# meyerls/PEGASUS

Hardware: AMD Instinct MI355X
Metric: rendered views/sec (RGB+depth+mask) on 2M-Gaussian scene @800x800 (higher is better)
Workload: dtype f32

## Files before the change

### pegasus_amd/csrc/preprocess.hip.h

```cpp
#pragma once
#include "blockcull.hip.h"
#include "pgr_common.h"

namespace pgr {

__device__ __forceinline__ float dot3_chain(float a0, float b0, float a1, float b1, float a2, float b2) {
    return fmaf(a2, b2, fmaf(a1, b1, a0 * b0));
}

__device__ __forceinline__ int clamp_trunc(float f, int hi) {
    if (!(f > 0.0f)) return 0;
    if (f >= (float)hi) return hi;
    return (int)f;
}

struct TileRect { int minx, miny, maxx, maxy; };

__device__ __forceinline__ TileRect tile_rect(float px, float py, int radius, int grid_x, int grid_y) {
    const float rf = (float)radius;
    TileRect r;
    r.minx = clamp_trunc((px - rf) / (float)TILE, grid_x);
    r.miny = clamp_trunc((py - rf) / (float)TILE, grid_y);
    r.maxx = clamp_trunc((px + rf + (float)(TILE - 1)) / (float)TILE, grid_x);
    r.maxy = clamp_trunc((py + rf + (float)(TILE - 1)) / (float)TILE, grid_y);
    return r;
}

__device__ __forceinline__ void cov3d_from_scale_rot(float s0, float s1, float s2, float mod, float4 q, float cov[6]) {
    const float r = q.x, x = q.y, y = q.z, z = q.w;
    float R[3][3];
    R[0][0] = 1.0f - 2.0f * (y * y + z * z);
    R[0][1] = 2.0f * (x * y - r * z);
    R[0][2] = 2.0f * (x * z + r * y);
    R[1][0] = 2.0f * (x * y + r * z);
    R[1][1] = 1.0f - 2.0f * (x * x + z * z);
    R[1][2] = 2.0f * (y * z - r * x);
    R[2][0] = 2.0f * (x * z - r * y);
    R[2][1] = 2.0f * (y * z + r * x);
    R[2][2] = 1.0f - 2.0f * (x * x + y * y);
    const float sx = mod * s0, sy = mod * s1, sz = mod * s2;
    float M[3][3];
#pragma unroll
    for (int i = 0; i < 3; ++i) {
        M[i][0] = R[i][0] * sx;
        M[i][1] = R[i][1] * sy;
        M[i][2] = R[i][2] * sz;
    }
    cov[0] = dot3_chain(M[0][0], M[0][0], M[0][1], M[0][1], M[0][2], M[0][2]);
    cov[1] = dot3_chain(M[0][0], M[1][0], M[0][1], M[1][1], M[0][2], M[1][2]);
    cov[2] = dot3_chain(M[0][0], M[2][0], M[0][1], M[2][1], M[0][2], M[2][2]);
    cov[3] = dot3_chain(M[1][0], M[1][0], M[1][1], M[1][1], M[1][2], M[1][2]);
    cov[4] = dot3_chain(M[1][0], M[2][0], M[1][1], M[2][1], M[1][2], M[2][2]);
    cov[5] = dot3_chain(M[2][0], M[2][0], M[2][1], M[2][1], M[2][2], M[2][2]);
}

template <int DEG>
__device__ __forceinline__ void sh_basis(float x, float y, float z, float b[16]) {
    constexpr float C0 = 0.28209479177387814f;
    constexpr float C1 = 0.4886025119029199f;
    constexpr float C2_0 = 1.0925484305920792f, C2_1 = -1.0925484305920792f, C2_2 = 0.31539156525252005f,
                    C2_3 = -1.0925484305920792f, C2_4 = 0.5462742152960396f;
    constexpr float C3_0 = -0.5900435899266435f, C3_1 = 2.890611442640554f, C3_2 = -0.4570457994644658f,
                    C3_3 = 0.3731763325901154f, C3_4 = -0.4570457994644658f, C3_5 = 1.445305721320277f,
                    C3_6 = -0.5900435899266435f;
    b[0] = C0;
    if constexpr (DEG > 0) {
        b[1] = -(C1 * y);
        b[2] = C1 * z;
        b[3] = -(C1 * x);
    }
    if constexpr (DEG > 1) {
        const float xx = x * x, yy = y * y, zz = z * z;
        const float xy = x * y, yz = y * z, xz = x * z;
        b[4] = C2_0 * xy;
        b[5] = C2_1 * yz;
        b[6] = C2_2 * (2.0f * zz - xx - yy);
        b[7] = C2_3 * xz;
        b[8] = C2_4 * (xx - yy);
        if constexpr (DEG > 2) {
            b[9] = C3_0 * y * (3.0f * xx - yy);
            b[10] = C3_1 * xy * z;
            b[11] = C3_2 * y * (4.0f * zz - xx - yy);
            b[12] = C3_3 * z * (2.0f * zz - 3.0f * xx - 3.0f * yy);
            b[13] = C3_4 * x * (4.0f * zz - xx - yy);
            b[14] = C3_5 * z * (xx - yy);
            b[15] = C3_6 * x * (xx - 3.0f * yy);
        }
    }
}

template <int DEG>
__device__ __forceinline__ float3 sh_to_rgb(const float* __restrict__ sh, float dx, float dy, float dz) {
    float b[16];
    sh_basis<DEG>(dx, dy, dz, b);
    constexpr int NC = (DEG + 1) * (DEG + 1);
    float acc[3];
    acc[0] = b[0] * sh[0];
    acc[1] = b[0] * sh[1];
    acc[2] = b[0] * sh[2];
#pragma unroll
    for (int k = 1; k < NC; ++k) {
        acc[0] = fmaf(b[k], sh[3 * k + 0], acc[0]);
        acc[1] = fmaf(b[k], sh[3 * k + 1], acc[1]);
        acc[2] = fmaf(b[k], sh[3 * k + 2], acc[2]);
    }
    return make_float3(fmaxf(acc[0] + 0.5f, 0.0f), fmaxf(acc[1] + 0.5f, 0.0f), fmaxf(acc[2] + 0.5f, 0.0f));
}

__device__ __forceinline__ uint2 candidate_rect(const TileRect& r, float mx, float my, float c_xx, float c_yy,
                                                float con_x, float con_y, float con_z, float opacity, int radius) {
    if (opacity < ALPHA_MIN) return make_uint2(0u, 0u);
    const uint2 full = make_uint2((uint32_t)r.minx | ((uint32_t)r.miny << 16), (uint32_t)r.maxx | ((uint32_t)r.maxy << 16));
    if (!(con_x > 0.0f) || !(con_z > 0.0f)) return full;
    const float t = 255.0f * opacity;
    const uint32_t bits = __float_as_uint(t);
    const float e = (float)((int)((bits >> 23) & 0xffu) - 127);
    const float m = __uint_as_float((bits & 0x007fffffu) | 0x3f800000u);
    const float tau = 1.3862944f * (e + (m - 1.0f) + 0.0861f);
    const float D = (float)radius + 2.0f * (float)TILE;
    const float M = (con_x + 2.0f * fabsf(con_y) + con_z) * D * D;
    const float tau2 = 1.001f * (tau + 0.00001f * M + 0.01f) + 0.001f;
    const float ex = sqrtf(tau2 * c_xx) * 1.001f + 1.0f, ey = sqrtf(tau2 * c_yy) * 1.001f + 1.0f;
    if (!(ex < 1.0e9f) || !(ey < 1.0e9f)) return full;
    const int minx = max(r.minx, (int)floorf((mx - ex - (float)(TILE - 1)) / (float)TILE) + 0);
    const int miny = max(r.miny, (int)floorf((my - ey - (float)(TILE - 1)) / (float)TILE) + 0);
    const int maxx = min(r.maxx, (int)floorf((mx + ex) / (float)TILE) + 1);
    const int maxy = min(r.maxy, (int)floorf((my + ey) / (float)TILE) + 1);
    if (maxx <= minx || maxy <= miny) return make_uint2(0u, 0u);
    return make_uint2((uint32_t)minx | ((uint32_t)miny << 16), (uint32_t)maxx | ((uint32_t)maxy << 16));
}

constexpr int SPLAT_F4 = 3;

struct PreOut {
    float4* splats;
    uint2* rects;
    uint2* crects;
    int32_t* radii;
};

struct ShRegs { float v[48]; };

template <int DEG>
__device__ __forceinline__ float3 sh_regs_to_rgb(const ShRegs& sh, float dx, float dy, float dz) {
    float b[16];
    sh_basis<DEG>(dx, dy, dz, b);
    constexpr int NC = (DEG + 1) * (DEG + 1);
    float acc[3];
    acc[0] = b[0] * sh.v[0];
    acc[1] = b[0] * sh.v[1];
    acc[2] = b[0] * sh.v[2];
#pragma unroll
    for (int k = 1; k < NC; ++k) {
        acc[0] = fmaf(b[k], sh.v[3 * k + 0], acc[0]);
        acc[1] = fmaf(b[k], sh.v[3 * k + 1], acc[1]);
        acc[2] = fmaf(b[k], sh.v[3 * k + 2], acc[2]);
    }
    return make_float3(fmaxf(acc[0] + 0.5f, 0.0f), fmaxf(acc[1] + 0.5f, 0.0f), fmaxf(acc[2] + 0.5f, 0.0f));
}

template <int DEG>
__device__ __forceinline__ void load_sh(ShRegs& sh, const float* __restrict__ p, bool vec4) {
    constexpr int NF = 3 * (DEG + 1) * (DEG + 1);
    if (vec4 && NF % 4 == 0) {
#pragma unroll
        for (int k = 0; k < NF / 4; ++k) {
            const float4 q = reinterpret_cast<const float4*>(p)[k];
            sh.v[4 * k + 0] = q.x; sh.v[4 * k + 1] = q.y; sh.v[4 * k + 2] = q.z; sh.v[4 * k + 3] = q.w;
        }
    } else {
#pragma unroll
        for (int k = 0; k < NF; ++k) sh.v[k] = p[k];
    }
}

typedef float f32x3_a4 __attribute__((ext_vector_type(3), aligned(4)));
typedef float f32x4_a4 __attribute__((ext_vector_type(4), aligned(4)));
template <int DEG>
__device__ __forceinline__ void load_sh_split(ShRegs& sh, const float* __restrict__ dc, const float* __restrict__ rest) {
    constexpr int NR = 3 * ((DEG + 1) * (DEG + 1) - 1);
    const f32x3_a4 c0 = *reinterpret_cast<const f32x3_a4*>(dc);
    sh.v[0] = c0.x; sh.v[1] = c0.y; sh.v[2] = c0.z;
#pragma unroll
    for (int k = 0; k < NR / 4; ++k) {
        const f32x4_a4 q = *reinterpret_cast<const f32x4_a4*>(rest + 4 * k);
        sh.v[3 + 4 * k + 0] = q.x; sh.v[3 + 4 * k + 1] = q.y; sh.v[3 + 4 * k + 2] = q.z; sh.v[3 + 4 * k + 3] = q.w;
    }
#pragma unroll
    for (int k = NR / 4 * 4; k < NR; ++k) sh.v[3 + k] = rest[k];
}

constexpr int POSE_STRIDE = 20;
struct PosedDev {
    const int32_t* object_id;
    const float* poses;
    int32_t k;
};

struct LayerDev {
    const int32_t* layer_id;
    int32_t n_layers;
};

template <int DEG, bool POSED, bool LAYERED = false, bool SPLIT_SH = false>
__global__ __launch_bounds__(PRE_BLOCK) __attribute__((amdgpu_waves_per_eu(4, 4))) void preprocess_batch_kernel(PgrScene sc, const CameraDev* __restrict__ cams,
                                                                     const PreOut* __restrict__ outs, int n_views,
                                                                     PosedDev posed, uint32_t* __restrict__ vis_out,
                                                                     int vis_words, LayerDev layers = LayerDev{nullptr, 0},
                                                                     int views_per_block = 0x7fffffff) {
    const int i = blockIdx.x * PRE_BLOCK + threadIdx.x;
    const int lane = threadIdx.x & (WAVE - 1);
    if (i - lane >= sc.n) return;
    const bool real = i < sc.n;
    const int group = __builtin_amdgcn_readfirstlane(i / WAVE);
    BlockBounds bounds;
    if (vis_out) bounds = wave_block_bounds(sc, i, real, POSED ? posed.object_id : nullptr);
    unsigned long long vis_mask = ~0ull;
    const float bx = real ? sc.means3d[3 * i + 0] : 0.f, by = real ? sc.means3d[3 * i + 1] : 0.f,
                bz = real ? sc.means3d[3 * i + 2] : 0.f;
    const int oid = POSED && real ? posed.object_id[i] : 0;
    int layer = 0;
    if (LAYERED && real) {
        layer = layers.layer_id[i];
        if (layer < 0 || layer > layers.n_layers) layer = 0;
    }
    float cov[6];
    bool have_cov = false, have_sh = false;
    ShRegs sh;
    const bool vec4 = (sc.sh_stride * 3) % 4 == 0 && (reinterpret_cast<uintptr_t>(sc.shs) & 15u) == 0;

    const int v_begin = (int)blockIdx.y * views_per_block;
    const int v_end = (int)min((long long)n_views, (long long)v_begin + views_per_block);
    for (int v = v_begin; v < v_end; ++v) {
        const CameraDev& cam = cams[v];
        const PreOut& o = outs[v];
        if (vis_out) {
            if ((v & (WAVE - 1)) == 0) {
                const int view = v + lane;
                vis_mask = __ballot(view < n_views && !block_is_culled(bounds, cams[view]));
                if (lane == 0) {
                    vis_out[(size_t)group * vis_words + (v >> 5)] = (uint32_t)vis_mask;
                    if ((v >> 5) + 1 < vis_words) vis_out[(size_t)group * vis_words + (v >> 5) + 1] = (uint32_t)(vis_mask >> 32);
                }
            }
            if (!((vis_mask >> (v & (WAVE - 1))) & 1ull)) {
                if (real && o.radii) o.radii[i] = 0;
                if (real && o.rects) o.rects[i] = make_uint2(0u, 0u);
                continue;
            }
        }
        if (!real) continue;
        if (LAYERED && layer == 0) {
            if (o.radii) o.radii[i] = 0;
            if (o.rects) o.rects[i] = make_uint2(0u, 0u);
            o.crects[i] = make_uint2(0u, 0u);
            continue;
        }
        int radius = 0;
        uint2 rect = make_uint2(0u, 0u), crect = make_uint2(0u, 0u);
        float vm[16];
#pragma unroll
        for (int k = 0; k < 16; ++k) vm[k] = cam.view[k];
        const float* pm = cam.proj;
        float cam_cx = cam.campos[0], cam_cy = cam.campos[1], cam_cz = cam.campos[2];
        float cam_tanx = cam.tanfovx, cam_tany = cam.tanfovy, cam_fx = cam.focal_x, cam_fy = cam.focal_y;
        int cam_w = cam.width, cam_h = cam.height, cam_gx = cam.grid_x, cam_gy = cam.grid_y;
        float4* out_splats = o.splats;
        uint2* out_crects = o.crects;
        asm volatile("" : "+s"(out_splats), "+s"(out_crects));
#pragma unroll
        for (int k = 0; k < 15; ++k)
            if ((k & 3) != 3) asm volatile("" : "+s"(vm[k]));
        asm volatile("" : "+s"(cam_cx), "+s"(cam_cy), "+s"(cam_cz), "+s"(cam_tanx), "+s"(cam_tany), "+s"(cam_fx), "+s"(cam_fy));
        asm volatile("" : "+s"(cam_w), "+s"(cam_h), "+s"(cam_gx), "+s"(cam_gy));
        float px = bx, py = by, pz = bz;
        const float* P = nullptr;
        if (POSED && oid > 0) {
            P = posed.poses + ((size_t)v * posed.k + (size_t)(oid - 1)) * POSE_STRIDE;
            const float dx = bx - P[12], dy = by - P[13], dz = bz - P[14];
            px = fmaf(P[2], dz, fmaf(P[1], dy, P[0] * dx)) + P[12] + P[9];
            py = fmaf(P[5], dz, fmaf(P[4], dy, P[3] * dx)) + P[13] + P[10];
            pz = fmaf(P[8], dz, fmaf(P[7], dy, P[6] * dx)) + P[14] + P[11];
        }
        float tx = vm[0] * px + vm[4] * py + vm[8] * pz + vm[12];
        float ty = vm[1] * px + vm[5] * py + vm[9] * pz + vm[13];
        const float tz = vm[2] * px + vm[6] * py + vm[10] * pz + vm[14];
        if (tz > NEAR_Z) {
            const float hx = pm[0] * px + pm[4] * py + pm[8] * pz + pm[12];
            const float hy = pm[1] * px + pm[5] * py + pm[9] * pz + pm[13];
            const float hw = pm[3] * px + pm[7] * py + pm[11] * pz + pm[15];
            const float p_w = 1.0f / (hw + 0.0000001f);
            const float ndc_x = hx * p_w, ndc_y = hy * p_w;
            if (POSED && P) {
                const float4 q = reinterpret_cast<const float4*>(sc.rotations)[i];
                const float inv = 1.0f / fmaxf(sqrtf(q.x * q.x + q.y * q.y + q.z * q.z + q.w * q.w), 1e-12f);
                const float w = q.x * inv, x = q.y * inv, y = q.z * inv, z = q.w * inv;
                const float a = P[15], b = P[16], c = P[17], d = P[18];
                const float4 qp = make_float4(a * w - b * x - c * y - d * z, a * x + b * w + c * z - d * y,
                                              a * y - b * z + c * w + d * x, a * z + b * y - c * x + d * w);
                cov3d_from_scale_rot(sc.scales[3 * i + 0], sc.scales[3 * i + 1], sc.scales[3 * i + 2],
                                     sc.scale_modifier, qp, cov);
            } else if (!have_cov) {
                if (sc.cov3d_precomp) {
#pragma unroll
                    for (int k = 0; k < 6; ++k) cov[k] = sc.cov3d_precomp[6 * (size_t)i + k];
                } else {
                    const float4 q = reinterpret_cast<const float4*>(sc.rotations)[i];
                    cov3d_from_scale_rot(sc.scales[3 * i + 0], sc.scales[3 * i + 1], sc.scales[3 * i + 2],
                                         sc.scale_modifier, q, cov);
                }
                have_cov = true;
            }
            const float limx = 1.3f * cam_tanx, limy = 1.3f * cam_tany;
            const float txtz = tx / tz, tytz = ty / tz;
            tx = fminf(limx, fmaxf(-limx, txtz)) * tz;
            ty = fminf(limy, fmaxf(-limy, tytz)) * tz;
            const float j00 = cam_fx / tz;
            const float j02 = -(cam_fx * tx) / (tz * tz);
            const float j11 = cam_fy / tz;
            const float j12 = -(cam_fy * ty) / (tz * tz);
            float T0[3], T1[3];
#pragma unroll
            for (int c = 0; c < 3; ++c) {
                T0[c] = fmaf(j02, vm[4 * c + 2], j00 * vm[4 * c + 0]);
                T1[c] = fmaf(j12, vm[4 * c + 2], j11 * vm[4 * c + 1]);
            }
            const float S[3][3] = {{cov[0], cov[1], cov[2]}, {cov[1], cov[3], cov[4]}, {cov[2], cov[4], cov[5]}};
            float U0[3], U1[3];
#pragma unroll
            for (int c = 0; c < 3; ++c) {
                U0[c] = dot3_chain(T0[0], S[0][c], T0[1], S[1][c], T0[2], S[2][c]);
                U1[c] = dot3_chain(T1[0], S[0][c], T1[1], S[1][c], T1[2], S[2][c]);
            }
            const float c_xx = dot3_chain(U0[0], T0[0], U0[1], T0[1], U0[2], T0[2]) + LOWPASS;
            const float c_xy = dot3_chain(U0[0], T1[0], U0[1], T1[1], U0[2], T1[2]);
            const float c_yy = dot3_chain(U1[0], T1[0], U1[1], T1[1], U1[2], T1[2]) + LOWPASS;
            const float det = c_xx * c_yy - c_xy * c_xy;
            if (det != 0.0f) {
                const float det_inv = 1.0f / det;
                const float con_x = c_yy * det_inv, con_y = -c_xy * det_inv, con_z = c_xx * det_inv;
                const float mid = 0.5f * (c_xx + c_yy);
                const float disc = sqrtf(fmaxf(0.1f, mid * mid - det));
                const float lambda1 = mid + disc, lambda2 = mid - disc;
                const float rad_f = ceilf(3.0f * sqrtf(fmaxf(lambda1, lambda2)));
                const int rad = rad_f >= 2147483520.0f ? 2147483520 : (int)rad_f;
                const float pix_x = ((ndc_x + 1.0f) * (float)cam_w - 1.0f) * 0.5f;
                const float pix_y = ((ndc_y + 1.0f) * (float)cam_h - 1.0f) * 0.5f;
                const TileRect r = tile_rect(pix_x, pix_y, rad, cam_gx, cam_gy);
                const int w = r.maxx - r.minx, h = r.maxy - r.miny;
                if (w > 0 && h > 0) {
                    float3 rgb;
                    if (sc.colors_precomp) {
                        rgb = make_float3(sc.colors_precomp[3 * (size_t)i], sc.colors_precomp[3 * (size_t)i + 1],
                                          sc.colors_precomp[3 * (size_t)i + 2]);
                    } else {
                        if (!have_sh) {
                            if constexpr (SPLIT_SH)
                                load_sh_split<DEG>(sh, sc.shs + (size_t)i * 3, sc.shs_rest + (size_t)i * (sc.sh_stride - 1) * 3);
                            else
                                load_sh<DEG>(sh, sc.shs + (size_t)i * sc.sh_stride * 3, vec4);
                            have_sh = true;
                        }
                        float dx = px - cam_cx, dy = py - cam_cy, dz = pz - cam_cz;
                        const float len = sqrtf(dx * dx + dy * dy + dz * dz);
                        dx = dx / len; dy = dy / len; dz = dz / len;
                        if (POSED && P) {
                            const float ox = fmaf(P[6], dz, fmaf(P[3], dy, P[0] * dx));
                            const float oy = fmaf(P[7], dz, fmaf(P[4], dy, P[1] * dx));
                            const float oz = fmaf(P[8], dz, fmaf(P[5], dy, P[2] * dx));
                            dx = ox; dy = oy; dz = oz;
                        }
                        rgb = sh_regs_to_rgb<DEG>(sh, dx, dy, dz);
                    }
                    radius = rad;
                    rect = make_uint2((uint32_t)r.minx | ((uint32_t)r.miny << 16),
                                      (uint32_t)r.maxx | ((uint32_t)r.maxy << 16));
                    const float op = sc.opacities[i];
                    crect = candidate_rect(r, pix_x, pix_y, c_xx, c_yy, con_x, con_y, con_z, op, rad);
                    if (LAYERED) {
                        const uint32_t off = (uint32_t)((layer - 1) * cam_gy) << 16;
                        rect.x += off; rect.y += off;
                        if (crect.x | crect.y) { crect.x += off; crect.y += off; }
                    }
                    float4* rec = out_splats + (size_t)i * SPLAT_F4;
                    rec[0] = make_float4(pix_x, pix_y, con_x, con_y);
                    rec[1] = make_float4(con_z, op, con_y / con_z, con_y / con_x);
                    rec[2] = make_float4(rgb.x, rgb.y, rgb.z, tz);
                }
            }
        }
        if (o.radii) o.radii[i] = radius;
        if (o.rects) o.rects[i] = rect;
        out_crects[i] = crect;
    }
}

constexpr int CAM_PACK_MAX = 32;
struct CamPack {
    const float* view[CAM_PACK_MAX];
    const float* proj[CAM_PACK_MAX];
    const float* campos[CAM_PACK_MAX];
    const float* bg[CAM_PACK_MAX];
    float tanfovx[CAM_PACK_MAX], tanfovy[CAM_PACK_MAX];
    int32_t depth_mode[CAM_PACK_MAX];
};

__device__ __forceinline__ void pack_camera(const CamPack& p, int v, int t, int width, int height, CameraDev* __restrict__ out) {
    if (t < 16) {
        out->view[t] = p.view[v][t];
        out->proj[t] = p.proj[v][t];
    }
    if (t < 3) {
        out->campos[t] = p.campos[v][t];
        out->bg[t] = p.bg[v][t];
    }
    if (t == 0) {
        const float tanfovx = p.tanfovx[v], tanfovy = p.tanfovy[v];
        out->tanfovx = tanfovx;
        out->tanfovy = tanfovy;
        out->focal_x = (float)width / (2.0f * tanfovx);
        out->focal_y = (float)height / (2.0f * tanfovy);
        out->width = width;
        out->height = height;
        out->grid_x = (width + TILE - 1) / TILE;
        out->grid_y = (height + TILE - 1) / TILE;
        out->depth_mode = p.depth_mode[v];
    }
}

__global__ void pack_camera_kernel(CamPack p, int width, int height, CameraDev* __restrict__ outs) {
    pack_camera(p, (int)blockIdx.x, (int)threadIdx.x, width, height, outs + blockIdx.x);
}

__global__ void mark_visible_kernel(int n, const float* __restrict__ means3d, const float* __restrict__ vm,
                                    uint8_t* __restrict__ present) {
    const int i = blockIdx.x * blockDim.x + threadIdx.x;
    if (i >= n) return;
    const float px = means3d[3 * i], py = means3d[3 * i + 1], pz = means3d[3 * i + 2];
    const float tz = vm[2] * px + vm[6] * py + vm[10] * pz + vm[14];
    present[i] = tz > NEAR_Z ? 1 : 0;
}

}
```

Baseline: 6199.

## Process visible views in pairs per Gaussian in preprocess kernel

Restructures the per-view loop in the preprocess kernel. It walks 64-view chunks using the wave-uniform visibility mask, skipping culled views through bit iteration instead of per-view branching, and projects two visible views per iteration to expose more instruction-level parallelism. The opacity load is hoisted and the SH load is deferred until at least one view is seen. This raises register pressure under a fixed waves-per-eu target and makes control flow more complex.

```diff
diff --git a/pegasus_amd/csrc/preprocess.hip.h b/pegasus_amd/csrc/preprocess.hip.h
--- a/pegasus_amd/csrc/preprocess.hip.h
+++ b/pegasus_amd/csrc/preprocess.hip.h
@@ -202,7 +202,239 @@
     int32_t n_layers;
 };
 
-template <int DEG, bool POSED, bool LAYERED = false, bool SPLIT_SH = false>
+struct ViewCam {
+    float vm[16];
+    const float* pm;
+    float cx, cy, cz, tanx, tany, fx, fy;
+    int w, h, gx, gy;
+    float4* splats;
+    uint2* crects;
+    uint2* rects;
+    int32_t* radii;
+};
+
+__device__ __forceinline__ void fetch_view_cam(ViewCam& c, const CameraDev& cam, const PreOut& o) {
+#pragma unroll
+    for (int k = 0; k < 16; ++k) c.vm[k] = cam.view[k];
+    c.pm = cam.proj;
+    c.cx = cam.campos[0]; c.cy = cam.campos[1]; c.cz = cam.campos[2];
+    c.tanx = cam.tanfovx; c.tany = cam.tanfovy; c.fx = cam.focal_x; c.fy = cam.focal_y;
+    c.w = cam.width; c.h = cam.height; c.gx = cam.grid_x; c.gy = cam.grid_y;
+    c.splats = o.splats;
+    c.crects = o.crects;
+    c.rects = o.rects;
+    c.radii = o.radii;
+    asm volatile("" : "+s"(c.splats), "+s"(c.crects));
+#pragma unroll
+    for (int k = 0; k < 15; ++k)
+        if ((k & 3) != 3) asm volatile("" : "+s"(c.vm[k]));
+    asm volatile("" : "+s"(c.cx), "+s"(c.cy), "+s"(c.cz), "+s"(c.tanx), "+s"(c.tany), "+s"(c.fx), "+s"(c.fy));
+    asm volatile("" : "+s"(c.w), "+s"(c.h), "+s"(c.gx), "+s"(c.gy));
+}
+
+struct ViewOut {
+    int radius;
+    uint2 rect, crect;
+};
+
+template <int NV, int DEG, bool POSED, bool LAYERED, bool SPLIT_SH>
+__device__ __forceinline__ void project_views(const PgrScene& sc, int i, bool vec4, const ViewCam (&c)[NV],
+                                              const float* const (&P)[NV], float bx, float by, float bz, float op, int layer,
+                                              float (&cov)[6], bool& have_cov, ShRegs& sh, bool& have_sh,
+                                              ViewOut (&out)[NV]) {
+    float px[NV], py[NV], pz[NV], tx[NV], ty[NV], tz[NV];
+    bool near_ok[NV], any_near = false;
+#pragma unroll
+    for (int k = 0; k < NV; ++k) {
+        const float* vm = c[k].vm;
+        px[k] = bx; py[k] = by; pz[k] = bz;
+        if (POSED && P[k]) {
+            const float dx = bx - P[k][12], dy = by - P[k][13], dz = bz - P[k][14];
+            px[k] = fmaf(P[k][2], dz, fmaf(P[k][1], dy, P[k][0] * dx)) + P[k][12] + P[k][9];
+            py[k] = fmaf(P[k][5], dz, fmaf(P[k][4], dy, P[k][3] * dx)) + P[k][13] + P[k][10];
+            pz[k] = fmaf(P[k][8], dz, fmaf(P[k][7], dy, P[k][6] * dx)) + P[k][14] + P[k][11];
+        }
+        tx[k] = vm[0] * px[k] + vm[4] * py[k] + vm[8] * pz[k] + vm[12];
+        ty[k] = vm[1] * px[k] + vm[5] * py[k] + vm[9] * pz[k] + vm[13];
+        tz[k] = vm[2] * px[k] + vm[6] * py[k] + vm[10] * pz[k] + vm[14];
+        near_ok[k] = tz[k] > NEAR_Z;
+        any_near |= near_ok[k];
+    }
+    if (!any_near) return;
+
+    float ndc_x[NV], ndc_y[NV], c_xx[NV], c_xy[NV], c_yy[NV], det[NV];
+    bool det_ok[NV], any_det = false;
+    if (!POSED || !P[0]) {
+        if (!have_cov) {
+            if (sc.cov3d_precomp) {
+#pragma unroll
+                for (int k = 0; k < 6; ++k) cov[k] = sc.cov3d_precomp[6 * (size_t)i + k];
+            } else {
+                const float4 q = reinterpret_cast<const float4*>(sc.rotations)[i];
+                cov3d_from_scale_rot(sc.scales[3 * i + 0], sc.scales[3 * i + 1], sc.scales[3 * i + 2],
+                                     sc.scale_modifier, q, cov);
+            }
+            have_cov = true;
+        }
+    }
+#pragma unroll
+    for (int k = 0; k < NV; ++k) {
+        const float* vm = c[k].vm;
+        const float* pm = c[k].pm;
+        const float hx = pm[0] * px[k] + pm[4] * py[k] + pm[8] * pz[k] + pm[12];
+        const float hy = pm[1] * px[k] + pm[5] * py[k] + pm[9] * pz[k] + pm[13];
+        const float hw = pm[3] * px[k] + pm[7] * py[k] + pm[11] * pz[k] + pm[15];
+        const float p_w = 1.0f / (hw + 0.0000001f);
+        ndc_x[k] = hx * p_w; ndc_y[k] = hy * p_w;
+        float cv[6];
+#pragma unroll
+        for (int j = 0; j < 6; ++j) cv[j] = cov[j];
+        if (POSED && P[k]) {
+            const float4 q = reinterpret_cast<const float4*>(sc.rotations)[i];
+            const float inv = 1.0f / fmaxf(sqrtf(q.x * q.x + q.y * q.y + q.z * q.z + q.w * q.w), 1e-12f);
+            const float w = q.x * inv, x = q.y * inv, y = q.z * inv, z = q.w * inv;
+            const float a = P[k][15], b = P[k][16], c4 = P[k][17], d = P[k][18];
+            const float4 qp = make_float4(a * w - b * x - c4 * y - d * z, a * x + b * w + c4 * z - d * y,
+                                          a * y - b * z + c4 * w + d * x, a * z + b * y - c4 * x + d * w);
+            cov3d_from_scale_rot(sc.scales[3 * i + 0], sc.scales[3 * i + 1], sc.scales[3 * i + 2],
+                                 sc.scale_modifier, qp, cv);
+        }
+        const float limx = 1.3f * c[k].tanx, limy = 1.3f * c[k].tany;
+        const float txtz = tx[k] / tz[k], tytz = ty[k] / tz[k];
+        tx[k] = fminf(limx, fmaxf(-limx, txtz)) * tz[k];
+        ty[k] = fminf(limy, fmaxf(-limy, tytz)) * tz[k];
+        const float j00 = c[k].fx / tz[k];
+        const float j02 = -(c[k].fx * tx[k]) / (tz[k] * tz[k]);
+        const float j11 = c[k].fy / tz[k];
+        const float j12 = -(c[k].fy * ty[k]) / (tz[k] * tz[k]);
+        float T0[3], T1[3];
+#pragma unroll
+        for (int a = 0; a < 3; ++a) {
+            T0[a] = fmaf(j02, vm[4 * a + 2], j00 * vm[4 * a + 0]);
+            T1[a] = fmaf(j12, vm[4 * a + 2], j11 * vm[4 * a + 1]);
+        }
+        const float S[3][3] = {{cv[0], cv[1], cv[2]}, {cv[1], cv[3], cv[4]}, {cv[2], cv[4], cv[5]}};
+        float U0[3], U1[3];
+#pragma unroll
+        for (int a = 0; a < 3; ++a) {
+            U0[a] = dot3_chain(T0[0], S[0][a], T0[1], S[1][a], T0[2], S[2][a]);
+            U1[a] = dot3_chain(T1[0], S[0][a], T1[1], S[1][a], T1[2], S[2][a]);
+        }
+        c_xx[k] = dot3_chain(U0[0], T0[0], U0[1], T0[1], U0[2], T0[2]) + LOWPASS;
+        c_xy[k] = dot3_chain(U0[0], T1[0], U0[1], T1[1], U0[2], T1[2]);
+        c_yy[k] = dot3_chain(U1[0], T1[0], U1[1], T1[1], U1[2], T1[2]) + LOWPASS;
+        det[k] = c_xx[k] * c_yy[k] - c_xy[k] * c_xy[k];
+        det_ok[k] = near_ok[k] && det[k] != 0.0f;
+        any_det |= det_ok[k];
+    }
+    if (!any_det) return;
+
+    float con_x[NV], con_y[NV], con_z[NV], pix_x[NV], pix_y[NV];
+    int rad[NV];
+    TileRect r[NV];
+    bool seen[NV], any_seen = false;
+#pragma unroll
+    for (int k = 0; k < NV; ++k) {
+        const float det_inv = 1.0f / det[k];
+        con_x[k] = c_yy[k] * det_inv; con_y[k] = -c_xy[k] * det_inv; con_z[k] = c_xx[k] * det_inv;
+        const float mid = 0.5f * (c_xx[k] + c_yy[k]);
+        const float disc = sqrtf(fmaxf(0.1f, mid * mid - det[k]));
+        const float lambda1 = mid + disc, lambda2 = mid - disc;
+        const float rad_f = ceilf(3.0f * sqrtf(fmaxf(lambda1, lambda2)));
+        rad[k] = rad_f >= 2147483520.0f ? 2147483520 : (int)rad_f;
+        pix_x[k] = ((ndc_x[k] + 1.0f) * (float)c[k].w - 1.0f) * 0.5f;
+        pix_y[k] = ((ndc_y[k] + 1.0f) * (float)c[k].h - 1.0f) * 0.5f;
+        r[k] = tile_rect(pix_x[k], pix_y[k], rad[k], c[k].gx, c[k].gy);
+        const int w = r[k].maxx - r[k].minx, h = r[k].maxy - r[k].miny;
+        seen[k] = det_ok[k] && w > 0 && h > 0;
+        any_seen |= seen[k];
+    }
+    if (!any_seen) return;
+
+#pragma unroll
+    for (int k = 0; k < NV; ++k) {
+        if (!seen[k]) continue;
+        out[k].radius = rad[k];
+        out[k].rect = make_uint2((uint32_t)r[k].minx | ((uint32_t)r[k].miny << 16),
+                                 (uint32_t)r[k].maxx | ((uint32_t)r[k].maxy << 16));
+        out[k].crect = candidate_rect(r[k], pix_x[k], pix_y[k], c_xx[k], c_yy[k], con_x[k], con_y[k], con_z[k], op, rad[k]);
+        if (LAYERED) {
+            const uint32_t off = (uint32_t)((layer - 1) * c[k].gy) << 16;
+            out[k].rect.x += off; out[k].rect.y += off;
+            if (out[k].crect.x | out[k].crect.y) { out[k].crect.x += off; out[k].crect.y += off; }
+        }
+        float4* rec = c[k].splats + (size_t)i * SPLAT_F4;
+        rec[0] = make_float4(pix_x[k], pix_y[k], con_x[k], con_y[k]);
+        rec[1] = make_float4(con_z[k], op, con_y[k] / con_z[k], con_y[k] / con_x[k]);
+    }
+    if (!sc.colors_precomp && !have_sh) {
+        if constexpr (SPLIT_SH)
+            load_sh_split<DEG>(sh, sc.shs + (size_t)i * 3, sc.shs_rest + (size_t)i * (sc.sh_stride - 1) * 3);
+        else
+            load_sh<DEG>(sh, sc.shs + (size_t)i * sc.sh_stride * 3, vec4);
+        have_sh = true;
+    }
+#pragma unroll
+    for (int k = 0; k < NV; ++k) {
+        if (!seen[k]) continue;
+        float3 rgb;
+        if (sc.colors_precomp) {
+            rgb = make_float3(sc.colors_precomp[3 * (size_t)i], sc.colors_precomp[3 * (size_t)i + 1],
+                              sc.colors_precomp[3 * (size_t)i + 2]);
+        } else {
+            float dx = px[k] - c[k].cx, dy = py[k] - c[k].cy, dz = pz[k] - c[k].cz;
+            const float len = sqrtf(dx * dx + dy * dy + dz * dz);
+            dx = dx / len; dy = dy / len; dz = dz / len;
+            if (POSED && P[k]) {
+                const float ox = fmaf(P[k][6], dz, fmaf(P[k][3], dy, P[k][0] * dx));
+                const float oy = fmaf(P[k][7], dz, fmaf(P[k][4], dy, P[k][1] * dx));
+                const float oz = fmaf(P[k][8], dz, fmaf(P[k][5], dy, P[k][2] * dx));
+                dx = ox; dy = oy; dz = oz;
+            }
+            rgb = sh_regs_to_rgb<DEG>(sh, dx, dy, dz);
+        }
+        (c[k].splats + (size_t)i * SPLAT_F4)[2] = make_float4(rgb.x, rgb.y, rgb.z, tz[k]);
+    }
+}
+
+template <int NV, int DEG, bool POSED, bool LAYERED, bool SPLIT_SH>
+__device__ __forceinline__ void walk_views(const PgrScene& sc, const CameraDev* __restrict__ cams,
+                                           const PreOut* __restrict__ outs, const PosedDev& posed, const int (&v)[NV],
+                                           int i, bool real, bool live, bool vec4, float bx, float by, float bz, float op,
+                                           int oid,
+                                           int layer, float (&cov)[6], bool& have_cov, ShRegs& sh, bool& have_sh) {
+    ViewCam c[NV];
+#pragma unroll
+    for (int k = 0; k < NV; ++k) fetch_view_cam(c[k], cams[v[k]], outs[v[k]]);
+    if (!real) return;
+    ViewOut out[NV];
+#pragma unroll
+    for (int k = 0; k < NV; ++k) {
+        out[k].radius = 0;
+        out[k].rect = make_uint2(0u, 0u);
+        out[k].crect = make_uint2(0u, 0u);
+    }
+    if (live) {
+        const float* P[NV];
+#pragma unroll
+        for (int k = 0; k < NV; ++k)
+            P[k] = POSED && oid > 0 ? posed.poses + ((size_t)v[k] * posed.k + (size_t)(oid - 1)) * POSE_STRIDE : nullptr;
+        project_views<NV, DEG, POSED, LAYERED, SPLIT_SH>(sc, i, vec4, c, P, bx, by, bz, op, layer, cov, have_cov, sh, have_sh, out);
+    }
+#pragma unroll
+    for (int k = 0; k < NV; ++k) {
+        if (c[k].radii) c[k].radii[i] = out[k].radius;
+        if (c[k].rects) c[k].rects[i] = out[k].rect;
+        c[k].crects[i] = out[k].crect;
+    }
+}
+
+#ifndef PGR_PRE_PAIR
+#define PGR_PRE_PAIR 2
+#endif
+constexpr int PRE_PAIR = PGR_PRE_PAIR;
+
+template <int DEG, bool POSED, bool LAYERED = false, bool SPLIT_SH = false, int PAIR = POSED ? 1 : PRE_PAIR>
 __global__ __launch_bounds__(PRE_BLOCK) __attribute__((amdgpu_waves_per_eu(4, 4))) void preprocess_batch_kernel(PgrScene sc, const CameraDev* __restrict__ cams,
                                                                      const PreOut* __restrict__ outs, int n_views,
                                                                      PosedDev posed, uint32_t* __restrict__ vis_out,
@@ -215,183 +447,57 @@
     const int group = __builtin_amdgcn_readfirstlane(i / WAVE);
     BlockBounds bounds;
     if (vis_out) bounds = wave_block_bounds(sc, i, real, POSED ? posed.object_id : nullptr);
-    unsigned long long vis_mask = ~0ull;
     const float bx = real ? sc.means3d[3 * i + 0] : 0.f, by = real ? sc.means3d[3 * i + 1] : 0.f,
                 bz = real ? sc.means3d[3 * i + 2] : 0.f;
+    const float op = real ? sc.opacities[i] : 0.f;
     const int oid = POSED && real ? posed.object_id[i] : 0;
     int layer = 0;
     if (LAYERED && real) {
         layer = layers.layer_id[i];
         if (layer < 0 || layer > layers.n_layers) layer = 0;
     }
-    float cov[6];
+    const bool live = real && (!LAYERED || layer != 0);
+    float cov[6] = {0.f, 0.f, 0.f, 0.f, 0.f, 0.f};
     bool have_cov = false, have_sh = false;
     ShRegs sh;
     const bool vec4 = (sc.sh_stride * 3) % 4 == 0 && (reinterpret_cast<uintptr_t>(sc.shs) & 15u) == 0;
 
     const int v_begin = (int)blockIdx.y * views_per_block;
     const int v_end = (int)min((long long)n_views, (long long)v_begin + views_per_block);
-    for (int v = v_begin; v < v_end; ++v) {
-        const CameraDev& cam = cams[v];
-        const PreOut& o = outs[v];
+    for (int w0 = v_begin & ~(WAVE - 1); w0 < v_end; w0 += WAVE) {
+        const int lo = max(v_begin, w0) - w0, hi = min(v_end, w0 + WAVE) - w0;
+        unsigned long long todo = (hi >= WAVE ? ~0ull : (1ull << hi) - 1ull) & ~((1ull << lo) - 1ull);
         if (vis_out) {
-            if ((v & (WAVE - 1)) == 0) {
-                const int view = v + lane;
-                vis_mask = __ballot(view < n_views && !block_is_culled(bounds, cams[view]));
-                if (lane == 0) {
-                    vis_out[(size_t)group * vis_words + (v >> 5)] = (uint32_t)vis_mask;
-                    if ((v >> 5) + 1 < vis_words) vis_out[(size_t)group * vis_words + (v >> 5) + 1] = (uint32_t)(vis_mask >> 32);
-                }
+            const int view = w0 + lane;
+            const unsigned long long vis_mask = __ballot(view < n_views && !block_is_culled(bounds, cams[view]));
+            if (lane == 0) {
+                vis_out[(size_t)group * vis_words + (w0 >> 5)] = (uint32_t)vis_mask;
+                if ((w0 >> 5) + 1 < vis_words) vis_out[(size_t)group * vis_words + (w0 >> 5) + 1] = (uint32_t)(vis_mask >> 32);
             }
-            if (!((vis_mask >> (v & (WAVE - 1))) & 1ull)) {
+            unsigned long long zero = __ballot(view < n_views && (outs[view].radii || outs[view].rects)) & todo & ~vis_mask;
+            while (zero) {
+                const PreOut& o = outs[w0 + __builtin_ctzll(zero)];
+                zero &= zero - 1ull;
                 if (real && o.radii) o.radii[i] = 0;
                 if (real && o.rects) o.rects[i] = make_uint2(0u, 0u);
-                continue;
             }
-        }
-        if (!real) continue;
-        if (LAYERED && layer == 0) {
-            if (o.radii) o.radii[i] = 0;
-            if (o.rects) o.rects[i] = make_uint2(0u, 0u);
-            o.crects[i] = make_uint2(0u, 0u);
-            continue;
-        }
-        int radius = 0;
-        uint2 rect = make_uint2(0u, 0u), crect = make_uint2(0u, 0u);
-        float vm[16];
-#pragma unroll
-        for (int k = 0; k < 16; ++k) vm[k] = cam.view[k];
-        const float* pm = cam.proj;
-        float cam_cx = cam.campos[0], cam_cy = cam.campos[1], cam_cz = cam.campos[2];
-        float cam_tanx = cam.tanfovx, cam_tany = cam.tanfovy, cam_fx = cam.focal_x, cam_fy = cam.focal_y;
-        int cam_w = cam.width, cam_h = cam.height, cam_gx = cam.grid_x, cam_gy = cam.grid_y;
-        float4* out_splats = o.splats;
-        uint2* out_crects = o.crects;
-        asm volatile("" : "+s"(out_splats), "+s"(out_crects));
-#pragma unroll
-        for (int k = 0; k < 15; ++k)
-            if ((k & 3) != 3) asm volatile("" : "+s"(vm[k]));
-        asm volatile("" : "+s"(cam_cx), "+s"(cam_cy), "+s"(cam_cz), "+s"(cam_tanx), "+s"(cam_tany), "+s"(cam_fx), "+s"(cam_fy));
-        asm volatile("" : "+s"(cam_w), "+s"(cam_h), "+s"(cam_gx), "+s"(cam_gy));
-        float px = bx, py = by, pz = bz;
-        const float* P = nullptr;
-        if (POSED && oid > 0) {
-            P = posed.poses + ((size_t)v * posed.k + (size_t)(oid - 1)) * POSE_STRIDE;
-            const float dx = bx - P[12], dy = by - P[13], dz = bz - P[14];
-            px = fmaf(P[2], dz, fmaf(P[1], dy, P[0] * dx)) + P[12] + P[9];
-            py = fmaf(P[5], dz, fmaf(P[4], dy, P[3] * dx)) + P[13] + P[10];
-            pz = fmaf(P[8], dz, fmaf(P[7], dy, P[6] * dx)) + P[14] + P[11];
-        }
-        float tx = vm[0] * px + vm[4] * py + vm[8] * pz + vm[12];
-        float ty = vm[1] * px + vm[5] * py + vm[9] * pz + vm[13];
-        const float tz = vm[2] * px + vm[6] * py + vm[10] * pz + vm[14];
-        if (tz > NEAR_Z) {
-            const float hx = pm[0] * px + pm[4] * py + pm[8] * pz + pm[12];
-            const float hy = pm[1] * px + pm[5] * py + pm[9] * pz + pm[13];
-            const float hw = pm[3] * px + pm[7] * py + pm[11] * pz + pm[15];
-            const float p_w = 1.0f / (hw + 0.0000001f);
-            const float ndc_x = hx * p_w, ndc_y = hy * p_w;
-            if (POSED && P) {
-                const float4 q = reinterpret_cast<const float4*>(sc.rotations)[i];
-                const float inv = 1.0f / fmaxf(sqrtf(q.x * q.x + q.y * q.y + q.z * q.z + q.w * q.w), 1e-12f);
-                const float w = q.x * inv, x = q.y * inv, y = q.z * inv, z = q.w * inv;
-                const float a = P[15], b = P[16], c = P[17], d = P[18];
-                const float4 qp = make_float4(a * w - b * x - c * y - d * z, a * x + b * w + c * z - d * y,
-                                              a * y - b * z + c * w + d * x, a * z + b * y - c * x + d * w);
-                cov3d_from_scale_rot(sc.scales[3 * i + 0], sc.scales[3 * i + 1], sc.scales[3 * i + 2],
-                                     sc.scale_modifier, qp, cov);
-            } else if (!have_cov) {
-                if (sc.cov3d_precomp) {
-#pragma unroll
-                    for (int k = 0; k < 6; ++k) cov[k] = sc.cov3d_precomp[6 * (size_t)i + k];
-                } else {
-                    const float4 q = reinterpret_cast<const float4*>(sc.rotations)[i];
-                    cov3d_from_scale_rot(sc.scales[3 * i + 0], sc.scales[3 * i + 1], sc.scales[3 * i + 2],
-                                         sc.scale_modifier, q, cov);
-                }
-                have_cov = true;
-            }
-            const float limx = 1.3f * cam_tanx, limy = 1.3f * cam_tany;
-            const float txtz = tx / tz, tytz = ty / tz;
-            tx = fminf(limx, fmaxf(-limx, txtz)) * tz;
-            ty = fminf(limy, fmaxf(-limy, tytz)) * tz;
-            const float j00 = cam_fx / tz;
-            const float j02 = -(cam_fx * tx) / (tz * tz);
-            const float j11 = cam_fy / tz;
-            const float j12 = -(cam_fy * ty) / (tz * tz);
-            float T0[3], T1[3];
-#pragma unroll
-            for (int c = 0; c < 3; ++c) {
-                T0[c] = fmaf(j02, vm[4 * c + 2], j00 * vm[4 * c + 0]);
-                T1[c] = fmaf(j12, vm[4 * c + 2], j11 * vm[4 * c + 1]);
-            }
-            const float S[3][3] = {{cov[0], cov[1], cov[2]}, {cov[1], cov[3], cov[4]}, {cov[2], cov[4], cov[5]}};
-            float U0[3], U1[3];
-#pragma unroll
-            for (int c = 0; c < 3; ++c) {
-                U0[c] = dot3_chain(T0[0], S[0][c], T0[1], S[1][c], T0[2], S[2][c]);
-                U1[c] = dot3_chain(T1[0], S[0][c], T1[1], S[1][c], T1[2], S[2][c]);
-            }
-            const float c_xx = dot3_chain(U0[0], T0[0], U0[1], T0[1], U0[2], T0[2]) + LOWPASS;
-            const float c_xy = dot3_chain(U0[0], T1[0], U0[1], T1[1], U0[2], T1[2]);
-            const float c_yy = dot3_chain(U1[0], T1[0], U1[1], T1[1], U1[2], T1[2]) + LOWPASS;
-            const float det = c_xx * c_yy - c_xy * c_xy;
-            if (det != 0.0f) {
-                const float det_inv = 1.0f / det;
-                const float con_x = c_yy * det_inv, con_y = -c_xy * det_inv, con_z = c_xx * det_inv;
-                const float mid = 0.5f * (c_xx + c_yy);
-                const float disc = sqrtf(fmaxf(0.1f, mid * mid - det));
-                const float lambda1 = mid + disc, lambda2 = mid - disc;
-                const float rad_f = ceilf(3.0f * sqrtf(fmaxf(lambda1, lambda2)));
-                const int rad = rad_f >= 2147483520.0f ? 2147483520 : (int)rad_f;
-                const float pix_x = ((ndc_x + 1.0f) * (float)cam_w - 1.0f) * 0.5f;
-                const float pix_y = ((ndc_y + 1.0f) * (float)cam_h - 1.0f) * 0.5f;
-                const TileRect r = tile_rect(pix_x, pix_y, rad, cam_gx, cam_gy);
-                const int w = r.maxx - r.minx, h = r.maxy - r.miny;
-                if (w > 0 && h > 0) {
-                    float3 rgb;
-                    if (sc.colors_precomp) {
-                        rgb = make_float3(sc.colors_precomp[3 * (size_t)i], sc.colors_precomp[3 * (size_t)i + 1],
-                                          sc.colors_precomp[3 * (size_t)i + 2]);
-                    } else {
-                        if (!have_sh) {
-                            if constexpr (SPLIT_SH)
-                                load_sh_split<DEG>(sh, sc.shs + (size_t)i * 3, sc.shs_rest + (size_t)i * (sc.sh_stride - 1) * 3);
-                            else
-                                load_sh<DEG>(sh, sc.shs + (size_t)i * sc.sh_stride * 3, vec4);
-                            have_sh = true;
-                        }
-                        float dx = px - cam_cx, dy = py - cam_cy, dz = pz - cam_cz;
-                        const float len = sqrtf(dx * dx + dy * dy + dz * dz);
-                        dx = dx / len; dy = dy / len; dz = dz / len;
-                        if (POSED && P) {
-                            const float ox = fmaf(P[6], dz, fmaf(P[3], dy, P[0] * dx));
-                            const float oy = fmaf(P[7], dz, fmaf(P[4], dy, P[1] * dx));
-                            const float oz = fmaf(P[8], dz, fmaf(P[5], dy, P[2] * dx));
-                            dx = ox; dy = oy; dz = oz;
-                        }
-                        rgb = sh_regs_to_rgb<DEG>(sh, dx, dy, dz);
-                    }
-                    radius = rad;
-                    rect = make_uint2((uint32_t)r.minx | ((uint32_t)r.miny << 16),
-                                      (uint32_t)r.maxx | ((uint32_t)r.maxy << 16));
-                    const float op = sc.opacities[i];
-                    crect = candidate_rect(r, pix_x, pix_y, c_xx, c_yy, con_x, con_y, con_z, op, rad);
-                    if (LAYERED) {
-                        const uint32_t off = (uint32_t)((layer - 1) * cam_gy) << 16;
-                        rect.x += off; rect.y += off;
-                        if (crect.x | crect.y) { crect.x += off; crect.y += off; }
-                    }
-                    float4* rec = out_splats + (size_t)i * SPLAT_F4;
-                    rec[0] = make_float4(pix_x, pix_y, con_x, con_y);
-                    rec[1] = make_float4(con_z, op, con_y / con_z, con_y / con_x);
-                    rec[2] = make_float4(rgb.x, rgb.y, rgb.z, tz);
-                }
-            }
-        }
-        if (o.radii) o.radii[i] = radius;
-        if (o.rects) o.rects[i] = rect;
-        out_crects[i] = crect;
+            todo &= vis_mask;
+        }
+        while (PAIR > 1 && (todo & (todo - 1ull))) {
+            const int va = w0 + __builtin_ctzll(todo);
+            todo &= todo - 1ull;
+            const int vb = w0 + __builtin_ctzll(todo);
+            todo &= todo - 1ull;
+            const int v[2] = {va, vb};
+            walk_views<2, DEG, POSED, LAYERED, SPLIT_SH>(sc, cams, outs, posed, v, i, real, live, vec4, bx, by, bz, op, oid,
+                                                         layer, cov, have_cov, sh, have_sh);
+        }
+        while (todo) {
+            const int v[1] = {w0 + __builtin_ctzll(todo)};
+            todo &= todo - 1ull;
+            walk_views<1, DEG, POSED, LAYERED, SPLIT_SH>(sc, cams, outs, posed, v, i, real, live, vec4, bx, by, bz, op, oid,
+                                                         layer, cov, have_cov, sh, have_sh);
+        }
     }
 }
 
```

New measurement: 6181. Within noise of the previous version (-0.3%).
